# YihangChen-ee/CNC

Hardware: AMD Instinct MI355X
Metric: ray-samples/s/GPU (16Lx2^19xF8 grid) (higher is better)
Workload: dtype f32; 1 GPU; configs[1]: 800x800 rays/GPU marched (step 5e-3) through a 128^3 ball occupancy, every sample encoded fwd (sign bit plane) + bwd (STE mask) on the binarised 16Lx2^19xF8 hash grid; rays_per_gpu=640000, chunk=1048576, table_rows=6120776, n_features=8, levels=16

## Files before the change

cnc_amd/csrc/grid_encode_merge.hip:

```cpp
#include <cstdlib>

#include "common.hpp"
#include "encoder_common.hpp"

namespace cnc {

typedef float f32x4 __attribute__((ext_vector_type(4)));

#ifndef CNC_MERGE_TILE_WINDOW
#define CNC_MERGE_TILE_WINDOW 8192
#endif
#ifndef CNC_MERGE_TILE_SEGMENT
#define CNC_MERGE_TILE_SEGMENT 8
#endif
constexpr uint32_t kMergeTileWindow = CNC_MERGE_TILE_WINDOW, kMergeTileSegment = CNC_MERGE_TILE_SEGMENT;
#ifndef CNC_MERGE_TILE_MIN_RES
#define CNC_MERGE_TILE_MIN_RES 52
#endif
constexpr uint32_t kMergeTileMinRes = CNC_MERGE_TILE_MIN_RES;

template <uint32_t TW, uint32_t TS>
__global__ __launch_bounds__(1024) void k_merge_tile_order(const float* __restrict__ inputs, uint32_t N,
                                                           uint16_t* __restrict__ order)
{
    constexpr uint32_t MB = 1024;
    __shared__ uint32_t s_sort[2 * MB], s_cnt[MB / 64];
    const uint32_t base = blockIdx.x * TW;
    constexpr uint32_t kSegs = TW / TS, kTiles = TW / MB;
    constexpr uint32_t kPastEnd = 0x3FFFFFu, kUnusable = 0x3FFFFEu;
    static_assert(MB == 1024 && kSegs <= MB && kSegs * TS == TW && kTiles * MB == TW, "one segment per thread, 10 index bits");
    static_assert(TS >= 1 && TS <= 16 && (TS & (TS - 1)) == 0 && (kTiles & (kTiles - 1)) == 0 && kTiles <= 16,
                  "a tile is at least one wave of segments");
    const uint32_t tid = threadIdx.x, lane = tid & 63, wave = tid >> 6;
    const uint32_t n_in = min(N - base, TW), n_seg = div_up(n_in, TS);
    float ax[3] = {0.0f, 0.0f, 0.0f};
    if (n_in >= 2) {
        float cand[3][3], len[3];
#pragma unroll
        for (uint32_t k = 0; k < 3; k++) {
            const size_t a = (size_t)base + min(k * 11u, n_in - 2);
#pragma unroll
            for (uint32_t d = 0; d < 3; d++) cand[k][d] = inputs[(a + 1) * 3 + d] - inputs[a * 3 + d];
            len[k] = (cand[k][0] * cand[k][0] + cand[k][1] * cand[k][1]) + cand[k][2] * cand[k][2];
        }
        const bool m0 = len[0] <= len[1] ? (len[1] > len[2] && len[0] > len[2]) : len[0] <= len[2];
        const bool m2 = len[0] <= len[1] ? (len[1] > len[2] && len[0] <= len[2]) : (len[0] > len[2] && len[1] <= len[2]);
#pragma unroll
        for (uint32_t d = 0; d < 3; d++) ax[d] = m0 ? cand[0][d] : m2 ? cand[2][d] : cand[1][d];
    }
    uint32_t q = kPastEnd;
    if (tid < n_seg) {
        const size_t s = (size_t)base + min(tid * TS + TS / 2, n_in - 1);
        const float  x0 = inputs[s * 3], x1 = inputs[s * 3 + 1], x2 = inputs[s * 3 + 2];
        const float  dep = (x0 * ax[0] + x1 * ax[1]) + x2 * ax[2];
        const bool   usable = x0 >= 0 && x0 <= 1 && x1 >= 0 && x1 <= 1 && x2 >= 0 && x2 <= 1 && dep == dep;
        uint32_t     u = __float_as_uint(dep);
        u ^= (u >> 31) ? 0xFFFFFFFFu : 0x80000000u;
        q = usable ? min(u >> 10, kUnusable - 1) : kUnusable;
    }
    const uint32_t qp = (uint32_t)__shfl_up((int)q, 1);
    const uint64_t db = __ballot(lane != 0 && q < qp && qp < kUnusable);
    if (lane == 0) s_cnt[wave] = (uint32_t)__popcll(db);
    uint32_t key = q << 10 | tid;
#pragma unroll
    for (uint32_t k = 2; k <= 64; k <<= 1) {
        uint32_t o = (uint32_t)__shfl_xor((int)key, (int)(k - 1));
        key = (lane & (k >> 1)) == 0 ? min(key, o) : max(key, o);
#pragma unroll
        for (uint32_t s = k >> 2; s >= 1; s >>= 1) {
            o = (uint32_t)__shfl_xor((int)key, (int)s);
            key = (lane & s) == 0 ? min(key, o) : max(key, o);
        }
    }
    __syncthreads();
    uint32_t n_rays = 1;
#pragma unroll
    for (uint32_t w = 0; w < MB / 64; w++) n_rays += s_cnt[w];
    const uint32_t have = n_rays * kSegs * 5u, want = n_seg * 32u * 7u;
    uint32_t       n_sub = have < want ? 1u : have < 2 * want ? 2u : have < 4 * want ? 4u : have < 8 * want ? 8u : 16u;
    n_sub = min(n_sub, kTiles);
    const uint32_t sub_segs = kSegs / n_sub;
    uint32_t p = 0;
    auto cross = [&](uint32_t mask, uint32_t bit) {
        s_sort[p * MB + tid] = key;
        __syncthreads();
        const uint32_t o = s_sort[p * MB + (tid ^ mask)];
        key = (tid & bit) == 0 ? min(key, o) : max(key, o);
        p ^= 1;
    };
    for (uint32_t k = 128; k <= sub_segs; k <<= 1) {
        cross(k - 1, k >> 1);
        for (uint32_t s = k >> 2; s >= 64; s >>= 1) cross(s, s);
#pragma unroll
        for (uint32_t s = 32; s >= 1; s >>= 1) {
            const uint32_t o = (uint32_t)__shfl_xor((int)key, (int)s);
            key = (lane & s) == 0 ? min(key, o) : max(key, o);
        }
    }
    if (tid < kSegs) order[(size_t)blockIdx.x * kSegs + tid] = (uint16_t)(key & (MB - 1));
}

template <bool STE, uint32_t MB, uint32_t TW, uint32_t TS>
__global__ __launch_bounds__(MB) void k_grid_encode_bwd_merge(
    const float* __restrict__ grad, const float* __restrict__ inputs, const float* __restrict__ emb,
    const int32_t* __restrict__ offsets, const int32_t* __restrict__ resolutions,
    float* __restrict__ grad_emb, uint32_t N, const uint32_t* __restrict__ clip_count, FeatLayout lay,
    const uint16_t* __restrict__ tile_order)
{
    constexpr uint32_t kMB = MB;
    constexpr uint32_t kMW = kMB / 64;
    constexpr uint32_t kMSlots = kMB <= 512 ? 1024 : 2048;
    constexpr uint32_t D = 3, F = 8, END = 0x7FFu;
    static_assert(kMB <= 1024, "run records pack start (10 bits) / end (11) / next (11)");
    __shared__ __attribute__((aligned(16))) float s_w4[kMB][4];
    __shared__ float    s_g[kMB][F];
    __shared__ __attribute__((aligned(16))) uint4 s_u[kMB];
    uint64_t* const s_key = reinterpret_cast<uint64_t*>(s_u);
    uint32_t* const h_slot = reinterpret_cast<uint32_t*>(s_u) + 2 * kMB;
    static_assert(kMSlots * 4 <= kMB * 8, "hash table fits the second half of s_u");
    __shared__ uint16_t s_run_start[kMB + 1];
    __shared__ uint32_t l_head[kMB];
    __shared__ uint32_t s_run_rec[kMB];
    __shared__ uint32_t s_wave_heads[kMW], s_wave_claims[kMW];

    const uint32_t tid = threadIdx.x, lane = tid & 63, wave = __builtin_amdgcn_readfirstlane(tid >> 6);
    const bool     mask_on = STE && (clip_count == nullptr || *clip_count != 0);
    auto wave_prefix = [&](const uint32_t* counts, uint32_t& before, uint32_t& total) {
        static_assert(kMW == 8 || kMW == 16, "the counts of a block fit one DPP row");
        const uint32_t h = counts[lane & (kMW - 1)];
        uint32_t       x = h;
        x += (uint32_t)__builtin_amdgcn_update_dpp(0, (int)x, 0x111, 0xF, 0xF, true);
        x += (uint32_t)__builtin_amdgcn_update_dpp(0, (int)x, 0x112, 0xF, 0xF, true);
        x += (uint32_t)__builtin_amdgcn_update_dpp(0, (int)x, 0x114, 0xF, 0xF, true);
        x += (uint32_t)__builtin_amdgcn_update_dpp(0, (int)x, 0x118, 0xF, 0xF, true);
        before = (uint32_t)__builtin_amdgcn_readlane((int)(x - h), (int)wave);
        total = (uint32_t)__builtin_amdgcn_readlane((int)x, (int)(kMW - 1));
    };
    const uint32_t n_slots = lay.n_slots;
    const uint32_t chunk = blockIdx.x / n_slots;
    const uint32_t slot = n_slots - 1 - blockIdx.x % n_slots;
    uint32_t       b = chunk * kMB + tid;
    const uint32_t off = (uint32_t)offsets[slot];
    const uint32_t hs = (uint32_t)offsets[slot + 1] - off;
    const uint32_t R = (uint32_t)resolutions[slot];

    if constexpr (TW != 0) {
        if (R >= kMergeTileMinRes) {
            constexpr uint32_t kTiles = TW / kMB, kSegs = TW / TS;
            const uint32_t win = chunk / kTiles, at = chunk % kTiles * (kMB / TS) + tid / TS;
            b = win * TW + (uint32_t)tile_order[(size_t)win * kSegs + at] * TS + tid % TS;
        }
    }
    for (uint32_t i = tid; i < kMSlots; i += kMB) h_slot[i] = 0;
    l_head[tid] = END;

    uint64_t key = ~0ull;
    uint32_t validmask = 0;
    {
        float    x[D];
        if (b < N && load_point<D>(inputs, b, x)) {
            Corners<D, false> c;
            c.setup(x, R, hs, 0, nullptr);
            key = (uint64_t)c.cell[0] | (uint64_t)c.cell[1] << 16 | (uint64_t)c.cell[2] << 32;
            if (R > kCellKeyMaxRes) key = ~0ull;
            {
                const uint32_t x1 = min(c.cell[0] + 1, R - 1), y1 = min(c.cell[1] + 1, R - 1), z1 = min(c.cell[2] + 1, R - 1);
                auto           border = [&](uint32_t q) { return (q == 0) | (q == R - 1); };
                const uint32_t inv = (border(c.cell[0]) ? 0x55u : 0u) | (border(x1) ? 0xAAu : 0u) | (border(c.cell[1]) ? 0x33u : 0u)
                    | (border(y1) ? 0xCCu : 0u) | (border(c.cell[2]) ? 0x0Fu : 0u) | (border(z1) ? 0xF0u : 0u);
                validmask = inv ^ 0xFFu;
            }
            *reinterpret_cast<float4*>(s_w4[tid]) = make_float4(c.frac[0], c.frac[1], c.frac[2], c.wn_re);
            const float* gp = grad + feat_index(lay, slot, N, b, F);
            float        g0[4], g1[4];
            load_vec<4>(gp, g0);
            load_vec<4>(gp + 4, g1);
#pragma unroll
            for (uint32_t j = 0; j < 4; j++) {
                s_g[tid][j] = g0[j];
                s_g[tid][4 + j] = g1[j];
            }
        }
        s_key[tid] = key;
    }
    __syncthreads();

    const bool     head = tid == 0 || s_key[tid - 1] != key;
    const uint64_t hb = __ballot(head);
    if (lane == 0) s_wave_heads[wave] = (uint32_t)__popcll(hb);
    __syncthreads();
    uint32_t before, total;
    wave_prefix(s_wave_heads, before, total);
    const uint32_t my_run = before + (uint32_t)__popcll(hb & ((1ull << lane) - 1ull));
    if (head) s_run_start[my_run] = (uint16_t)tid;
    if (tid == 0) s_run_start[total] = (uint16_t)kMB;
    __syncthreads();

    bool     claimer = false;
    if (head && key != ~0ull) {
        uint32_t sl = (((uint32_t)key ^ (uint32_t)(key >> 16) ^ (uint32_t)(key >> 32)) * 2654435761u) >> (32 - __builtin_ctz(kMSlots));
        uint32_t rep;
        for (;;) {
            const uint32_t seen = atomicCAS(&h_slot[sl], 0u, my_run + 1);
            if (seen == 0) { claimer = true; rep = my_run; break; }
            rep = seen - 1;
            if (s_key[s_run_start[rep]] == key) break;
            sl = (sl + 1) & (kMSlots - 1);
        }
        const uint32_t next = atomicExch(&l_head[rep], my_run);
        s_run_rec[my_run] = tid | (uint32_t)s_run_start[my_run + 1] << 10 | next << 21;
    }
    const uint64_t cb = __ballot(claimer);
    if (lane == 0) s_wave_claims[wave] = (uint32_t)__popcll(cb);
    __syncthreads();
    uint32_t g_before, n_cells;
    wave_prefix(s_wave_claims, g_before, n_cells);
    uint4 my_cell = make_uint4(0, 0, 0, 0);
    if (claimer) my_cell = make_uint4(s_run_rec[l_head[my_run]], (uint32_t)key, (uint32_t)(key >> 32), validmask);
    if (claimer) s_u[g_before + (uint32_t)__popcll(cb & ((1ull << lane) - 1ull))] = my_cell;
    __syncthreads();

    const uint32_t c = lane / F, f = lane % F;
    const uint32_t mi = lane & 15u, mk = lane >> 4;
    const bool     half_b = (mi & 8u) != 0;
    const float    sx = (mi & 1u) ? 1.0f : -1.0f, ox = (mi & 1u) ? 0.0f : 1.0f;
    const float    sy = (mi & 2u) ? 1.0f : -1.0f, oy = (mi & 2u) ? 0.0f : 1.0f;
    const float    sz = (mi & 4u) ? 1.0f : -1.0f, oz = (mi & 4u) ? 0.0f : 1.0f;
    auto flush = [&](uint32_t row, float v) {
        const size_t at = (size_t)row * F + f;
        if (mask_on) {
            const float e = emb[at];
            if (!(e >= -1.0f && e <= 1.0f)) return;
        }
        unsafeAtomicAdd(grad_emb + at, v);
    };
    uint32_t stride = 1, sd[D];
#pragma unroll
    for (uint32_t d = 0; d < D; d++) {
        sd[d] = stride;
        if (stride <= hs) stride *= R;
    }
    const bool hashed = stride > hs, pow2 = (hs & (hs - 1)) == 0;
    constexpr uint32_t primes[3] = {1u, 2654435761u, 805459861u};
    const bool cx = (c & 1u) != 0, cy = (c & 2u) != 0, cz = (c & 4u) != 0;
    const uint32_t m1 = hashed ? primes[1] : sd[1], m2 = hashed ? primes[2] : sd[2];
    auto row_of = [&](uint32_t k_lo, uint32_t k_hi) -> uint32_t {
        const uint32_t gx = k_lo & 0xFFFFu, gy = k_lo >> 16, gz = k_hi & 0xFFFFu;
        const uint32_t x0 = gx, x1 = min(gx + 1, R - 1);
        const uint32_t y0 = gy * m1, y1 = min(gy + 1, R - 1) * m1;
        const uint32_t z0 = gz * m2, z1 = min(gz + 1, R - 1) * m2;
        const uint32_t px = cx ? x1 : x0, py = cy ? y1 : y0, pz = cz ? z1 : z0;
        uint32_t index = hashed ? (px ^ py ^ pz) : (px + py + pz);
        if (pow2) index &= hs - 1;
        else if (index >= hs) index %= hs;
        return off + index;
    };

    for (uint32_t g = wave; g < n_cells; g += kMW) {
        const uint4 cell = s_u[g];
        uint32_t    rec = __builtin_amdgcn_readfirstlane(cell.x);
        const uint32_t k_lo = __builtin_amdgcn_readfirstlane(cell.y);
        const uint32_t k_hi = __builtin_amdgcn_readfirstlane(cell.z);
        f32x4 S = {0.0f, 0.0f, 0.0f, 0.0f};
        for (;;) {
            uint32_t a0 = rec & 0x3FFu, a1 = (rec >> 10) & 0x7FFu, b0, b1, nxt = rec >> 21;
            if (nxt != END) {
                const uint32_t rb = __builtin_amdgcn_readfirstlane(s_run_rec[nxt]);
                b0 = rb & 0x3FFu, b1 = (rb >> 10) & 0x7FFu, nxt = rb >> 21;
            } else {
                b1 = a1;
                a1 = b0 = min(a1, a0 + ((((a1 - a0 + 1u) >> 1) + 3u) & ~3u));
            }
            const uint32_t steps = max(a1 - a0, b1 - b0);
            const uint32_t m0 = half_b ? b0 : a0, m1 = half_b ? b1 : a1;
            const uint32_t ahead = s_run_rec[nxt & (kMB - 1)];
            for (uint32_t p = 0; p < steps; p += 4) {
                const uint32_t ps = m0 + p + mk;
                float          a = 0.0f, bv = 0.0f;
                if (ps < m1) {
                    const float4 q = *reinterpret_cast<const float4*>(s_w4[ps]);
                    const float wx = __builtin_fmaf(q.x, sx, ox), wy = __builtin_fmaf(q.y, sy, oy),
                                wz = __builtin_fmaf(q.z, sz, oz);
                    a = ((wx * wy) * wz) * q.w;
                    bv = s_g[ps][mi & 7u];
                }
                S = __builtin_amdgcn_mfma_f32_16x16x4f32(a, bv, S, 0, 0, 0);
            }
            if (nxt == END) break;
            rec = __builtin_amdgcn_readfirstlane(ahead);
        }
        const int   src = (int)(f + 16u * (c >> 2));
        const float e0 = __shfl(S[0], src) + __shfl(S[0], src + 40), e1 = __shfl(S[1], src) + __shfl(S[1], src + 40),
                    e2 = __shfl(S[2], src) + __shfl(S[2], src + 40), e3 = __shfl(S[3], src) + __shfl(S[3], src + 40);
        if ((cell.w >> c) & 1u)
            flush(row_of(k_lo, k_hi), (c & 2u) ? ((c & 1u) ? e3 : e2) : ((c & 1u) ? e1 : e0));
    }
}

template <bool STE>
__global__ __launch_bounds__(256) void k_grid_encode_bwd_wide(
    const float* __restrict__ grad, const float* __restrict__ inputs, const float* __restrict__ emb,
    const int32_t* __restrict__ offsets, const int32_t* __restrict__ resolutions,
    float* __restrict__ grad_emb, uint32_t N, const uint32_t* __restrict__ clip_count, FeatLayout lay)
{
    constexpr uint32_t D = 3, F = 8, C = 8;
    const uint32_t slot = blockIdx.y;
    const uint32_t R = (uint32_t)resolutions[slot];
    if (R <= kCellKeyMaxRes) return;
    const bool     mask_on = STE && (clip_count == nullptr || *clip_count != 0);
    const uint32_t off = (uint32_t)offsets[slot];
    const uint32_t hs = (uint32_t)offsets[slot + 1] - off;
    for (uint32_t b = blockIdx.x * blockDim.x + threadIdx.x; b < N; b += gridDim.x * blockDim.x) {
        float x[D];
        if (load_point<D>(inputs, b, x)) {
            uint32_t cell[D];
            float    frac[D];
#pragma unroll
            for (uint32_t d = 0; d < D; d++) {
                float p = x[d] * (float)(R - 2);
                p = p + 0.5f;
                const float fl = floorf(p);
                cell[d] = (uint32_t)fl;
                frac[d] = p - fl;
            }
            uint32_t valid = 0;
            float    wn = 0;
#pragma unroll 1
            for (uint32_t i = 0; i < C; i++) {
                float wi = 1;
                bool  border = false;
#pragma unroll
                for (uint32_t d = 0; d < D; d++) {
                    const bool     bit = (i >> d) & 1u;
                    const uint32_t q = bit ? min(cell[d] + 1, R - 1) : cell[d];
                    wi *= bit ? frac[d] : 1 - frac[d];
                    border |= (q == 0) | (q == R - 1);
                }
                valid |= (border ? 0u : 1u) << i;
                wn += border ? 0.0f : wi;
            }
            if (wn == 0) wn = 1e-9f;
            const float* gp = grad + feat_index(lay, slot, N, b, F);
            float        g[F];
            bool         nonzero = false;
#pragma unroll
            for (uint32_t k = 0; k < F; k++) {
                g[k] = gp[k];
                nonzero |= g[k] != 0.0f;
            }
            if (nonzero) scatter_point<D, F>(cell, frac, valid, 1.0f / wn, off, hs, R, g, emb, grad_emb, mask_on);
        }
    }
}

uint64_t merge_tile_order_bytes(uint32_t N)
{
    return ((uint64_t)div_up(N, kMergeTileWindow) * (kMergeTileWindow / kMergeTileSegment) * 2 + 255) / 256 * 256;
}

void launch_bwd_merge(const EncoderCall& c)
{
    const uint32_t N = c.N, L = c.L;
    const bool     ste = c.ste();
    FeatLayout     lay = c.lay;
    lay.n_slots = L;
    const bool small = (uint64_t)div_up(N, 1024u) * L < 4096u;
#define CNC_MERGE_GO(ST, MBS, W, S)                                                                                     \
    hipLaunchKernelGGL((k_grid_encode_bwd_merge<ST, MBS, W, S>), dim3(div_up(N, MBS) * L), dim3(MBS), 0, c.stream, c.grad, \
                       c.inputs, c.emb, c.offsets, c.resolutions, c.out, N, c.clip_count, lay, c.tile_order)
    if (small) {
        if (ste) CNC_MERGE_GO(true, 512u, 0u, 0u);
        else CNC_MERGE_GO(false, 512u, 0u, 0u);
    } else if ((c.flags & CNC_FLAG_MERGE_CONSECUTIVE) || c.tile_order == nullptr) {
        if (ste) CNC_MERGE_GO(true, 1024u, 0u, 0u);
        else CNC_MERGE_GO(false, 1024u, 0u, 0u);
    } else {
        hipLaunchKernelGGL((k_merge_tile_order<kMergeTileWindow, kMergeTileSegment>), dim3(div_up(N, kMergeTileWindow)),
                           dim3(1024), 0, c.stream, c.inputs, N, c.tile_order);
        if (ste) CNC_MERGE_GO(true, 1024u, kMergeTileWindow, kMergeTileSegment);
        else CNC_MERGE_GO(false, 1024u, kMergeTileWindow, kMergeTileSegment);
    }
#undef CNC_MERGE_GO
    const dim3 wide(div_up(N, 256u) < 16u ? div_up(N, 256u) : 16u, L);
#define CNC_WIDE_GO(ST)                                                                                               \
    hipLaunchKernelGGL((k_grid_encode_bwd_wide<ST>), wide, dim3(256), 0, c.stream, c.grad, c.inputs, c.emb, c.offsets, \
                       c.resolutions, c.out, N, c.clip_count, lay)
    if (ste) CNC_WIDE_GO(true);
    else CNC_WIDE_GO(false);
#undef CNC_WIDE_GO
}

}
```

Before: 954.3 million ray-samples/s.

## Compact merged-cell samples contiguously and split cells into capped work units

Replaces the per-cell linked list of runs with a counting-sort compaction. Each sample's weights and gradients are scattered into contiguous shared-memory ranges per cell, and each cell becomes one or more work units capped at a fixed number of samples. Waves now pull units dynamically from a shared atomic counter instead of taking cells round-robin, so heavy cells stop serialising one wave while others sit idle. This costs an extra scatter pass, an extra barrier, and more shared-memory atomics, and a cell split across units issues several global flushes for the same rows.

```diff
diff --git a/cnc_amd/csrc/grid_encode_merge.hip b/cnc_amd/csrc/grid_encode_merge.hip
--- a/cnc_amd/csrc/grid_encode_merge.hip
+++ b/cnc_amd/csrc/grid_encode_merge.hip
@@ -18,6 +18,11 @@
 #define CNC_MERGE_TILE_MIN_RES 52
 #endif
 constexpr uint32_t kMergeTileMinRes = CNC_MERGE_TILE_MIN_RES;
+#ifndef CNC_MERGE_UNIT_CAP
+#define CNC_MERGE_UNIT_CAP 512
+#endif
+constexpr uint32_t kMergeUnitCap = CNC_MERGE_UNIT_CAP;
+static_assert(kMergeUnitCap >= 8 && kMergeUnitCap % 8 == 0, "whole steps of eight samples");
 
 template <uint32_t TW, uint32_t TS>
 __global__ __launch_bounds__(1024) void k_merge_tile_order(const float* __restrict__ inputs, uint32_t N,
@@ -110,8 +115,9 @@
     constexpr uint32_t kMB = MB;
     constexpr uint32_t kMW = kMB / 64;
     constexpr uint32_t kMSlots = kMB <= 512 ? 1024 : 2048;
-    constexpr uint32_t D = 3, F = 8, END = 0x7FFu;
-    static_assert(kMB <= 1024, "run records pack start (10 bits) / end (11) / next (11)");
+    constexpr uint32_t kCap = kMergeUnitCap;
+    constexpr uint32_t D = 3, F = 8;
+    static_assert(kMB <= 1024, "run records pack representative run / place in the cell / first thread, 10 bits each");
     __shared__ __attribute__((aligned(16))) float s_w4[kMB][4];
     __shared__ float    s_g[kMB][F];
     __shared__ __attribute__((aligned(16))) uint4 s_u[kMB];
@@ -119,9 +125,10 @@
     uint32_t* const h_slot = reinterpret_cast<uint32_t*>(s_u) + 2 * kMB;
     static_assert(kMSlots * 4 <= kMB * 8, "hash table fits the second half of s_u");
     __shared__ uint16_t s_run_start[kMB + 1];
-    __shared__ uint32_t l_head[kMB];
+    __shared__ uint32_t s_cell_n[kMB];
     __shared__ uint32_t s_run_rec[kMB];
-    __shared__ uint32_t s_wave_heads[kMW], s_wave_claims[kMW];
+    __shared__ uint32_t s_wave_heads[kMW];
+    __shared__ uint32_t s_ctr[2];
 
     const uint32_t tid = threadIdx.x, lane = tid & 63, wave = __builtin_amdgcn_readfirstlane(tid >> 6);
     const bool     mask_on = STE && (clip_count == nullptr || *clip_count != 0);
@@ -152,10 +159,13 @@
         }
     }
     for (uint32_t i = tid; i < kMSlots; i += kMB) h_slot[i] = 0;
-    l_head[tid] = END;
+    s_cell_n[tid] = 0;
+    if (tid < 2) s_ctr[tid] = tid == 0 ? 0u : kMW;
 
     uint64_t key = ~0ull;
     uint32_t validmask = 0;
+    float4   w4 = make_float4(0.0f, 0.0f, 0.0f, 0.0f);
+    float    g0[4] = {0.0f, 0.0f, 0.0f, 0.0f}, g1[4] = {0.0f, 0.0f, 0.0f, 0.0f};
     {
         float    x[D];
         if (b < N && load_point<D>(inputs, b, x)) {
@@ -170,16 +180,10 @@
                     | (border(y1) ? 0xCCu : 0u) | (border(c.cell[2]) ? 0x0Fu : 0u) | (border(z1) ? 0xF0u : 0u);
                 validmask = inv ^ 0xFFu;
             }
-            *reinterpret_cast<float4*>(s_w4[tid]) = make_float4(c.frac[0], c.frac[1], c.frac[2], c.wn_re);
+            w4 = make_float4(c.frac[0], c.frac[1], c.frac[2], c.wn_re);
             const float* gp = grad + feat_index(lay, slot, N, b, F);
-            float        g0[4], g1[4];
             load_vec<4>(gp, g0);
             load_vec<4>(gp + 4, g1);
-#pragma unroll
-            for (uint32_t j = 0; j < 4; j++) {
-                s_g[tid][j] = g0[j];
-                s_g[tid][4 + j] = g1[j];
-            }
         }
         s_key[tid] = key;
     }
@@ -191,7 +195,7 @@
     __syncthreads();
     uint32_t before, total;
     wave_prefix(s_wave_heads, before, total);
-    const uint32_t my_run = before + (uint32_t)__popcll(hb & ((1ull << lane) - 1ull));
+    const uint32_t my_run = before + (uint32_t)__popcll(hb & ((2ull << lane) - 1ull)) - 1u;
     if (head) s_run_start[my_run] = (uint16_t)tid;
     if (tid == 0) s_run_start[total] = (uint16_t)kMB;
     __syncthreads();
@@ -207,25 +211,39 @@
             if (s_key[s_run_start[rep]] == key) break;
             sl = (sl + 1) & (kMSlots - 1);
         }
-        const uint32_t next = atomicExch(&l_head[rep], my_run);
-        s_run_rec[my_run] = tid | (uint32_t)s_run_start[my_run + 1] << 10 | next << 21;
-    }
-    const uint64_t cb = __ballot(claimer);
-    if (lane == 0) s_wave_claims[wave] = (uint32_t)__popcll(cb);
-    __syncthreads();
-    uint32_t g_before, n_cells;
-    wave_prefix(s_wave_claims, g_before, n_cells);
-    uint4 my_cell = make_uint4(0, 0, 0, 0);
-    if (claimer) my_cell = make_uint4(s_run_rec[l_head[my_run]], (uint32_t)key, (uint32_t)(key >> 32), validmask);
-    if (claimer) s_u[g_before + (uint32_t)__popcll(cb & ((1ull << lane) - 1ull))] = my_cell;
-    __syncthreads();
+        const uint32_t len = (uint32_t)s_run_start[my_run + 1] - tid;
+        s_run_rec[my_run] = rep | atomicAdd(&s_cell_n[rep], len) << 10 | tid << 20;
+    }
+    __syncthreads();
+    if (claimer) {
+        const uint32_t n = s_cell_n[my_run], units = (n + kCap - 1) / kCap;
+        const uint32_t got = atomicAdd(&s_ctr[0], n | units << 16);
+        const uint32_t first = got & 0xFFFFu, end = first + n;
+        uint32_t       at = got >> 16;
+        s_cell_n[my_run] = first;
+        for (uint32_t p = first; p < end; p += kCap, at++)
+            s_u[at] = make_uint4(p | min(p + kCap, end) << 16, (uint32_t)key, (uint32_t)(key >> 32), validmask);
+    }
+    __syncthreads();
+    if (key != ~0ull) {
+        const uint32_t rr = s_run_rec[my_run];
+        const uint32_t at = s_cell_n[rr & 0x3FFu] + ((rr >> 10) & 0x3FFu) + (tid - (rr >> 20));
+        *reinterpret_cast<float4*>(s_w4[at]) = w4;
+#pragma unroll
+        for (uint32_t j = 0; j < 4; j++) {
+            s_g[at][j] = g0[j];
+            s_g[at][4 + j] = g1[j];
+        }
+    }
+    __syncthreads();
+    const uint32_t n_units = __builtin_amdgcn_readfirstlane(s_ctr[0]) >> 16;
 
     const uint32_t c = lane / F, f = lane % F;
     const uint32_t mi = lane & 15u, mk = lane >> 4;
-    const bool     half_b = (mi & 8u) != 0;
     const float    sx = (mi & 1u) ? 1.0f : -1.0f, ox = (mi & 1u) ? 0.0f : 1.0f;
     const float    sy = (mi & 2u) ? 1.0f : -1.0f, oy = (mi & 2u) ? 0.0f : 1.0f;
     const float    sz = (mi & 4u) ? 1.0f : -1.0f, oz = (mi & 4u) ? 0.0f : 1.0f;
+    const uint32_t mine = 2u * mk + ((mi >> 3) & 1u);
     auto flush = [&](uint32_t row, float v) {
         const size_t at = (size_t)row * F + f;
         if (mask_on) {
@@ -256,44 +274,33 @@
         return off + index;
     };
 
-    for (uint32_t g = wave; g < n_cells; g += kMW) {
+    for (uint32_t g = wave; g < n_units;) {
         const uint4 cell = s_u[g];
-        uint32_t    rec = __builtin_amdgcn_readfirstlane(cell.x);
+        const uint32_t span = __builtin_amdgcn_readfirstlane(cell.x);
         const uint32_t k_lo = __builtin_amdgcn_readfirstlane(cell.y);
         const uint32_t k_hi = __builtin_amdgcn_readfirstlane(cell.z);
+        const uint32_t p_end = span >> 16;
         f32x4 S = {0.0f, 0.0f, 0.0f, 0.0f};
-        for (;;) {
-            uint32_t a0 = rec & 0x3FFu, a1 = (rec >> 10) & 0x7FFu, b0, b1, nxt = rec >> 21;
-            if (nxt != END) {
-                const uint32_t rb = __builtin_amdgcn_readfirstlane(s_run_rec[nxt]);
-                b0 = rb & 0x3FFu, b1 = (rb >> 10) & 0x7FFu, nxt = rb >> 21;
-            } else {
-                b1 = a1;
-                a1 = b0 = min(a1, a0 + ((((a1 - a0 + 1u) >> 1) + 3u) & ~3u));
+        for (uint32_t p = span & 0xFFFFu; p < p_end; p += 8) {
+            const uint32_t ps = p + mine;
+            float          a = 0.0f, bv = 0.0f;
+            if (ps < p_end) {
+                const float4 q = *reinterpret_cast<const float4*>(s_w4[ps]);
+                const float wx = __builtin_fmaf(q.x, sx, ox), wy = __builtin_fmaf(q.y, sy, oy),
+                            wz = __builtin_fmaf(q.z, sz, oz);
+                a = ((wx * wy) * wz) * q.w;
+                bv = s_g[ps][mi & 7u];
             }
-            const uint32_t steps = max(a1 - a0, b1 - b0);
-            const uint32_t m0 = half_b ? b0 : a0, m1 = half_b ? b1 : a1;
-            const uint32_t ahead = s_run_rec[nxt & (kMB - 1)];
-            for (uint32_t p = 0; p < steps; p += 4) {
-                const uint32_t ps = m0 + p + mk;
-                float          a = 0.0f, bv = 0.0f;
-                if (ps < m1) {
-                    const float4 q = *reinterpret_cast<const float4*>(s_w4[ps]);
-                    const float wx = __builtin_fmaf(q.x, sx, ox), wy = __builtin_fmaf(q.y, sy, oy),
-                                wz = __builtin_fmaf(q.z, sz, oz);
-                    a = ((wx * wy) * wz) * q.w;
-                    bv = s_g[ps][mi & 7u];
-                }
-                S = __builtin_amdgcn_mfma_f32_16x16x4f32(a, bv, S, 0, 0, 0);
-            }
-            if (nxt == END) break;
-            rec = __builtin_amdgcn_readfirstlane(ahead);
-        }
+            S = __builtin_amdgcn_mfma_f32_16x16x4f32(a, bv, S, 0, 0, 0);
+        }
+        uint32_t taken = 0;
+        if (lane == 0) taken = atomicAdd(&s_ctr[1], 1u);
         const int   src = (int)(f + 16u * (c >> 2));
         const float e0 = __shfl(S[0], src) + __shfl(S[0], src + 40), e1 = __shfl(S[1], src) + __shfl(S[1], src + 40),
                     e2 = __shfl(S[2], src) + __shfl(S[2], src + 40), e3 = __shfl(S[3], src) + __shfl(S[3], src + 40);
         if ((cell.w >> c) & 1u)
             flush(row_of(k_lo, k_hi), (c & 2u) ? ((c & 1u) ? e3 : e2) : ((c & 1u) ? e1 : e0));
+        g = __builtin_amdgcn_readfirstlane(taken);
     }
 }
 
```

Result: faster. 988.7 million ray-samples/s, median of 6 (+3.6%).
